# PhilipWilliamVentura/multimodal-financial-analysis-tool-using-paligemma

Measured on AMD Instinct MI355X. Metric: decode tokens/sec per GPU + prefill ms (224px img + 32-tok prompt), PaliGemma-3B, higher is better.
Workload: dtype bf16; 1 GPU; configs[1]: paligemma-3b-pt-224 greedy KV-cached decode, batch 1, after a 256-image-token + 32-text-token prefill; batch_per_gpu=1, global_batch=1, prompt_len=288, images_gathered=1, parallelism=replicas x1 (weights RCCL-broadcast), hipgraph=True, steps_per_graph_launch=1

## Files before the change

### include/pgmi.h

```cpp
#ifndef PGMI_H
#define PGMI_H

#include <stddef.h>
#include <stdint.h>

#ifdef __cplusplus
extern "C" {
#endif

#define PGMI_OK 0
#define PGMI_E_ARG -1
#define PGMI_E_STATE -2
#define PGMI_E_HIP -3
#define PGMI_E_NOMEM -4

#define PGMI_DTYPE_BF16 0
#define PGMI_DTYPE_F16 1
#define PGMI_DTYPE_F32 2

typedef struct pgmi_ctx pgmi_ctx;

typedef struct pgmi_config {
    int v_hidden, v_intermediate, v_layers, v_heads, v_channels, v_image, v_patch;
    float v_ln_eps;
// ... 54 lines not shown
                           const void* position, int position_dtype, const void* mask, int mask_dtype,
                           int64_t mask_b_stride, float* logits, int64_t* next_ids, int use_graph, void* stream);
int pgmi_set_prefill_graph(pgmi_ctx* ctx, int on);
#define PGMI_GRAPH_CACHE_MAX 64
int pgmi_graph_count(const pgmi_ctx* ctx, int which);
int pgmi_set_decode_staged_norm(pgmi_ctx* ctx, int on);
int pgmi_lm_head(pgmi_ctx* ctx, const void* normed, int rows, float* logits, void* stream);
int pgmi_lm_final_hidden(pgmi_ctx* ctx, void* out, int rows, void* stream);

#define PGMI_COMM_ID_BYTES 128
int pgmi_comm_unique_id(void* id_out);
int pgmi_comm_init(int device, int nranks, int rank, const void* id, void** comm_out);
int pgmi_comm_destroy(void* comm);
int pgmi_broadcast_weights(pgmi_ctx* ctx, void* comm, int root, void* stream);

int pgmi_argmax(pgmi_ctx* ctx, const float* logits, int rows, int V, int64_t* out, void* stream);

int pgmi_eos_update(pgmi_ctx* ctx, int64_t* next_ids, int32_t* finished, int B, int64_t eos_id, int64_t pad_id,
                    int32_t* n_alive, void* stream);

int pgmi_decode_kernel(pgmi_ctx* ctx, int which, int layer, int B, void* stream);

int pgmi_preprocess(pgmi_ctx* ctx, const void* src_hwc, int H, int W, int out_h, int out_w, float* out_chw,
                    void* stream);

int pgmi_prefill_kernel(pgmi_ctx* ctx, int which, int layer, int rows, void* stream);

int pgmi_prefill_probe(pgmi_ctx* ctx, int on);
int pgmi_prefill_probe_times(pgmi_ctx* ctx, float* us, int n);
int pgmi_tune_gemm(int cfg, int split);
int pgmi_tune_gemm_shape(int M, int N, int K, int dual, int cfg, int split);

int pgmi_debug_gemm_tiles(int n_mt, int n_nt, int S, int BM, int BN, int K, int* mt, int* nt, int* z);

int pgmi_tune_attention(int variant);

int pgmi_sample_top_p(pgmi_ctx* ctx, const float* x, int rows, int V, float temperature, float top_p,
                      const float* u, int64_t* out, float* kept_mass, void* stream);

int pgmi_op_gemm(pgmi_ctx* ctx, const void* A, const void* W, int M, int N, int K, int epi, const void* bias,
                 const void* res, void* out, void* stream);
int pgmi_op_gemm_strided(pgmi_ctx* ctx, const void* A, int lda, const void* W, int ldw, int M, int N, int K, int epi,
                         const void* bias, const void* res, void* out, void* stream);
int pgmi_op_rmsnorm(pgmi_ctx* ctx, const void* x, const void* w, int rows, int D, float eps, void* out,
                    void* stream);
int pgmi_op_layernorm(pgmi_ctx* ctx, const void* x, const void* w, const void* b, int rows, int D, float eps,
                      void* out, void* stream);
int pgmi_op_add(pgmi_ctx* ctx, const void* a, const void* b, int64_t n, void* out, void* stream);
int pgmi_op_patch_embed(pgmi_ctx* ctx, const void* pixels, int pixel_dtype, int B, int C, int H, int P,
                        const void* conv_w, const void* conv_b, const void* pos, int D, void* out, void* stream);
int pgmi_op_attention(pgmi_ctx* ctx, const void* q, const void* k, const void* v, void* o, int B, int Lq, int Lk,
                      int H, int Hkv, int head_dim, float scale, void* stream);
int pgmi_op_attention_ex(pgmi_ctx* ctx, const void* q, const void* k, const void* v, void* o, int B, int Lq, int Lk,
                         int H, int Hkv, int head_dim, int kv_layout, float scale, int scale_div, const void* mask,
                         int mask_dtype, int64_t m_b_stride, int64_t m_h_stride, int64_t m_q_stride, void* probs,
                         void* stream);
int pgmi_op_rope(pgmi_ctx* ctx, const void* x, const void* cos_rows, const void* sin_rows, int64_t rows, int heads,
                 int head_dim, void* out, void* stream);
int pgmi_op_scale(pgmi_ctx* ctx, const void* x, float a, int64_t n, void* out, void* stream);
int pgmi_op_gemv_res(pgmi_ctx* ctx, const void* x, const void* W, int B, int N, int K, void* h_inout,
                     void* stream);

#ifdef __cplusplus
}
#endif
#endif
// ... 1 lines not shown
```

### multimodal-financial-analysis-tool-using-paligemma_amd/csrc/engine.hip

```cpp
#include <algorithm>
#include <cmath>
#include <cstdio>
#include <cstdlib>
#include <cstring>
#include <map>
#include <string>
#include <unordered_map>
#include <vector>

#include <dlfcn.h>

#include <rccl/rccl.h>

#include "../../include/pgmi.h"
#include "common.h"
#include "launch.h"
#include "safetensors_hdr.h"

using namespace pgmi;

static thread_local std::string g_err;

static int fail(int code, const std::string& msg) {
    g_err = msg;
// ... 1355 lines not shown
    if ((rc = ensure_prepared(x))) return rc;
    const pgmi_config& c = x->c;
    if (rows < 1 || rows > c.max_batch * c.max_seq) return fail(PGMI_E_ARG, "rows exceed the prefill workspace");
    if (layer < 0 || layer >= c.t_layers) return fail(PGMI_E_ARG, "layer out of range");
    hipStream_t s = (hipStream_t)stream;
    const int H = c.t_hidden;
    const TextLayerW& w = x->w.t[layer];
    switch (which) {
        case 0: {
            EpiArgs g{};
            g.out = x->ACT; g.ldo = c.t_intermediate;
            gemm(s, x->Tn, H, w.gate_up, H, rows, c.t_intermediate, H, EPI_GEGLU, g, x->ws, x->ws_bytes,
                 c.t_intermediate);
            break;
        }
        case 1: {
            EpiArgs d{};
            d.res = x->Hs; d.ldr = H; d.out = x->Hs; d.ldo = H;
            gemm(s, x->ACT, c.t_intermediate, w.down, c.t_intermediate, rows, H, c.t_intermediate, EPI_RES, d, x->ws,
                 x->ws_bytes, 0, true);
            break;
        }
        default: return fail(PGMI_E_ARG, "unknown kernel id");
    }
    LAUNCHCHK();
    return 0;
}

int pgmi_debug_gemm_tiles(int n_mt, int n_nt, int S, int BM, int BN, int K, int* mt, int* nt, int* z) {
    if (n_mt < 1 || n_nt < 1 || S < 1 || !mt || !nt || !z) return fail(PGMI_E_ARG, "bad argument");
    return gemm_tile_order(n_mt, n_nt, S, BM, BN, K, mt, nt, z);
}

int pgmi_tune_gemm(int cfg, int split) {
    if (cfg >= kGemmCfgs || split < 0 || split > 32) return fail(PGMI_E_ARG, "bad GEMM plan");
    gemm_force_plan(cfg, split);
    return 0;
}

int pgmi_tune_gemm_shape(int M, int N, int K, int dual, int cfg, int split) {
    if (cfg >= kGemmCfgs || split < 0 || split > 16) return fail(PGMI_E_ARG, "bad GEMM plan");
    if (gemm_force_shape(M, N, K, dual, cfg, split)) return fail(PGMI_E_ARG, "too many per-shape GEMM plans");
    return 0;
}

int pgmi_tune_attention(int variant) {
    static const int ok[] = {-1, 0, 7, 8, 41, 42, 21, 22, 44, 24, 9, 91, 92, 94, 81, 82};
    for (int v : ok)
        if (v == variant) {
            attention_force_variant(variant);
            return 0;
        }
    return fail(PGMI_E_ARG, "unknown attention variant");
}

int pgmi_sample_top_p(pgmi_ctx* x, const float* logits, int rows, int V, float temperature, float top_p,
                      const float* u, int64_t* out, float* kept_mass, void* stream) {
    if (!x || !logits || !u || !out) return fail(PGMI_E_ARG, "null argument");
    if (rows <= 0 || V <= 0) return fail(PGMI_E_ARG, "sample_top_p: empty probabilities");
    if (!(top_p >= 0.f)) return fail(PGMI_E_ARG, "sample_top_p: top_p must be >= 0");
    if (!x->ws) return fail(PGMI_E_STATE, "workspace not allocated (pgmi_prepare)");
    const int per = (int)std::min<size_t>((size_t)rows, x->ws_bytes / sample_scratch_bytes(1, V));
    if (per < 1) return fail(PGMI_E_ARG, "sample_top_p: vocabulary exceeds the scratch");
    for (int r0 = 0; r0 < rows; r0 += per) {
        const int nr = std::min(per, rows - r0);
        sample_top_p((hipStream_t)stream, logits + (size_t)r0 * V, nr, V, temperature, top_p, u + r0, x->ws,
// ... 185 lines not shown
```

### multimodal-financial-analysis-tool-using-paligemma_amd/csrc/kernels_gemm.hip

```cpp
#include <map>
#include <mutex>
#include <tuple>
#include <vector>

#include <hip/hip_ext.h>

#include "common.h"
#include "launch.h"

#include <cstdlib>
#include <type_traits>

namespace pgmi {

constexpr int BK = 64;
constexpr int LDSK = 72;

#ifndef PGMI_GEMM_DIAG
#define PGMI_GEMM_DIAG 0
#endif
template <int TM, int TN, int NB>
__device__ __forceinline__ void diag_consume(const short8 (&fa)[TM], const short8 (&fb)[NB][TN]) {
#pragma unroll
    for (int i = 0; i < TM; ++i) asm volatile("" ::"v"(fa[i]));
#pragma unroll
    for (int b = 0; b < NB; ++b)
#pragma unroll
        for (int j = 0; j < TN; ++j) asm volatile("" ::"v"(fb[b][j]));
}

template <int EPI>
__device__ __forceinline__ void epi_store(const EpiArgs& ea, int m, int n, float acc, float acc2) {
// ... 1024 lines not shown
    P288w = 6,
    P256w = 7,
    P352w = 8,
    P288n = 9,
    P256n = 10,
    P128w = 11,
    P288t = 12,
    P256t = 13,
    P64x64 = 14,
    P128x64 = 15,
    P64x128 = 16,
    P128x128 = 17,
    P64x64d = 18,
    P128x64d = 19,
    Q288w = 20,
    Q352w = 21,
    Q256w = 22,
    Q288x256 = 23,
    P64x64s3 = 24,
    P64x64s4 = 25,
    P32x64s4 = 26,
    P64x32s4 = 27,
    P96x64s4 = 28,
    P96x64s3 = 29,
    W288w = 30,
    W288n = 31,
    W64x64 = 32,
    W352w = 33,
    W128x128 = 34,
    W128x64 = 35,
    E256 = 36,
    E192 = 37,
    R288w = 38,
    kNumCfg = 39,
};
static_assert(kNumCfg == kGemmCfgs, "launch.h kGemmCfgs");

struct Plan {
    Cfg cfg;
    int bm, bn, split;
};

static int g_force_cfg = -1, g_force_split = 0;

void gemm_force_plan(int cfg, int split) {
    g_force_cfg = cfg;
    g_force_split = split;
}

struct ShapePlan {
    int M, N, K;
    bool dual;
    int cfg, split;
};
static ShapePlan g_shape_plans[16];
static int g_n_shape_plans = 0;

int gemm_force_shape(int M, int N, int K, int dual, int cfg, int split) {
    for (int i = 0; i < g_n_shape_plans; ++i)
        if (g_shape_plans[i].M == M && g_shape_plans[i].N == N && g_shape_plans[i].K == K &&
            g_shape_plans[i].dual == (dual != 0)) {
            g_shape_plans[i] = g_shape_plans[--g_n_shape_plans];
            break;
        }
    if (cfg < 0) return 0;
    if (g_n_shape_plans >= 16) return -1;
    g_shape_plans[g_n_shape_plans++] = {M, N, K, dual != 0, cfg, split < 1 ? 1 : split};
    return 0;
}

static Plan choose(int M, int N, int K, bool dual) {
    if (g_force_cfg >= 0) {
        static const int bms[] = {288, 288, 256, 256, 128, 128, 288, 256, 352, 288, 256, 128, 288, 256, 64, 128, 64, 128, 64, 128, 288, 352, 256, 288, 64, 64, 32, 64, 96, 96, 288, 288, 64, 352, 128, 128, 256, 192, 288};
        static const int bns[] = {64, 32, 64, 32, 128, 64, 128, 128, 128, 64, 64, 128, 32, 32, 64, 64, 128, 128, 64, 64, 128, 128, 128, 256, 64, 64, 64, 32, 64, 64, 128, 64, 64, 128, 128, 64, 256, 256, 128};
        const int c = g_force_cfg;
        const int bn = (dual && c >= P288w) ? bns[c] / 2 : bns[c];
        return {(Cfg)c, bms[c], bn, dual && c < P288w ? 1 : (g_force_split > 0 ? g_force_split : 1)};
    }
    struct Entry { int M, N, K; bool dual; Cfg cfg; int split; };
    static const Entry table[] = {
        {288, 2560, 2048, false, W64x64, 1},
        {288, 2048, 2048, false, W128x128, 4},
        {288, 16384, 2048, true, R288w, 1},
        {288, 2048, 16384, false, W288n, 8},
        {256, 3456, 1152, false, P64x64s4, 1},
        {256, 1152, 1152, false, P64x64s4, 3},
        {256, 4304, 1152, false, P96x64s4, 1},
        {256, 1152, 4304, false, P96x64s4, 4},
        {256, 1152, 640, false, P64x32s4, 1},
        {256, 2048, 1152, false, P32x64s4, 1},
        {1056, 2560, 2048, false, W128x128, 1},
        {1056, 2048, 2048, false, W128x128, 1},
        {1056, 16384, 2048, true, E192, 1},
        {1056, 2048, 16384, false, E192, 5},
        {1024, 3456, 1152, false, W128x128, 1},
        {1024, 1152, 1152, false, P96x64s4, 1},
        {1024, 4304, 1152, false, W288w, 1},
        {1024, 1152, 4304, false, W128x128, 3},
        {2048, 3456, 1152, false, W288w, 1},
        {2048, 1152, 1152, false, W128x128, 1},
        {2048, 4304, 1152, false, W352w, 1},
        {2048, 1152, 4304, false, W288w, 2},
        {2048, 2048, 1152, false, W128x128, 1},
        {2304, 2560, 2048, false, Q256w, 1},
        {2304, 2048, 2048, false, W288n, 1},
        {2304, 16384, 2048, true, E256, 1},
        {2304, 2048, 16384, false, W288w, 2},
    };
    static const int bms[] = {288, 288, 256, 256, 128, 128, 288, 256, 352, 288, 256, 128, 288, 256, 64, 128, 64, 128, 64, 128, 288, 352, 256, 288, 64, 64, 32, 64, 96, 96, 288, 288, 64, 352, 128, 128, 256, 192, 288};
    static const int bns[] = {64, 32, 64, 32, 128, 64, 128, 128, 128, 64, 64, 128, 32, 32, 64, 64, 128, 128, 64, 64, 128, 128, 128, 256, 64, 64, 64, 32, 64, 64, 128, 64, 64, 128, 128, 64, 256, 256, 128};
    auto mk = [&](Cfg c, int split) -> Plan { return {c, bms[c], dual ? bns[c] / 2 : bns[c], dual ? 1 : split}; };
    for (int i = 0; i < g_n_shape_plans; ++i) {
        const ShapePlan& o = g_shape_plans[i];
        if (o.M == M && o.N == N && o.K == K && o.dual == dual) return mk((Cfg)o.cfg, o.split);
    }
    for (const Entry& e : table)
        if (e.M == M && e.N == N && e.K == K && e.dual == dual) return mk(e.cfg, e.split);
    if (M <= 16) {
        if (dual) return mk(P64x128, 1);
        if (K >= 8192) return mk(P64x64, 8);
    }
    if (dual) return mk(M <= 288 || M >= 2048 ? W288w : W352w, 1);
    if (K >= 8192) return mk(M <= 288 ? W288n : W288w, M <= 288 ? 8 : M <= 1056 ? 4 : 2);
    const long t64 = (long)((M + 63) / 64) * ((N + 63) / 64);
    if (t64 <= 256) return mk(P64x64, 1);
    const long t128 = (long)((M + 127) / 128) * ((N + 127) / 128);
    Plan p = mk(P128w, 1);
    const int nkt = (K + 63) / 64;
    while (t128 * p.split < 200 && p.split < 4 && nkt / (p.split * 2) >= 4) p.split *= 2;
    return p;
}

size_t gemm_ws_bytes(int M, int N, int K) {
    Plan p = choose(M, N, K, false);
    return p.split > 1 ? (size_t)p.split * M * N * sizeof(float) : 0;
}

static int xcd_block_pick(int n_mt, int n_nt, int S, int BM, int BN, int K);
static int xcd_block(int n_mt, int n_nt, int S, int BM, int BN, int K) {
    static std::mutex mu;
    static std::map<std::tuple<int, int, int, int, int, int>, int> memo;
    const auto key = std::make_tuple(n_mt, n_nt, S, BM, BN, K);
    std::lock_guard<std::mutex> lock(mu);
    auto it = memo.find(key);
    if (it != memo.end()) return it->second;
    const int code = xcd_block_pick(n_mt, n_nt, S, BM, BN, K);
    memo[key] = code;
    return code;
}

static int xcd_block_pick(int n_mt, int n_nt, int S, int BM, int BN, int K) {
    const long G = (long)n_mt * n_nt * S;
    if ((long)n_mt * BM < 2048) return 0;
    if (G % 8 != 0 || n_mt >= 64 * 8 || G > 65536) return 0;
    const double ks = (double)K / S * 2.0;
    const long q = G / 8;
    double run = 0.0;
    for (int x = 0; x < 8; ++x) {
        long na = 0, nb = 0;
        std::vector<char> sa((size_t)n_mt * S, 0), sb((size_t)n_nt * S, 0);
        for (long idx = x * q; idx < (x + 1) * q; ++idx) {
            const int mt = (int)(idx % n_mt), z = (int)((idx / n_mt) % S), nt = (int)(idx / ((long)n_mt * S));
            if (!sa[(size_t)mt * S + z]++) ++na;
            if (!sb[(size_t)nt * S + z]++) ++nb;
        }
        run += ks * ((double)na * BM + (double)nb * BN);
    }
    double best = 0.8 * run;
// ... 80 lines not shown
    const int n_mt = (M + BM - 1) / BM, n_nt = (N + BN - 1) / BN;
    dim3 grid(n_mt * n_nt, split);
    const int code = xcd_block(n_mt, n_nt, split, BM, NB * BN, K);
    static bool attr_set = false;
    if (!attr_set) {
        (void)hipFuncSetAttribute(reinterpret_cast<const void*>(&k_gemm_p<NW, WM, TM, TN, NB, STQ, EK, false>),
                                  hipFuncAttributeMaxDynamicSharedMemorySize, (int)lds);
        (void)hipFuncSetAttribute(reinterpret_cast<const void*>(&k_gemm_p<NW, WM, TM, TN, NB, STQ, EK, true>),
                                  hipFuncAttributeMaxDynamicSharedMemorySize, (int)lds);
        attr_set = true;
    }
    if (EPI < 0 || split > 1) {
        PGMI_GEMM_LAUNCH((k_gemm_p<NW, WM, TM, TN, NB, STQ, EK, true>), grid, dim3(64 * NW), lds, s, A, lda, W, ldw, M, N, K, per,
                           ea, ws, up_off, n_mt, code);
        if (EPI >= 0) {
            long total4 = ((long)M * N + 3) / 4;
            long blocks = (total4 + 255) / 256;
            if (blocks > 4096) blocks = 4096;
            hipLaunchKernelGGL((k_splitk_epi<EK>), dim3((unsigned)blocks), dim3(256), 0, s, ws, split, M, N, ea);
        }
    } else {
        PGMI_GEMM_LAUNCH((k_gemm_p<NW, WM, TM, TN, NB, STQ, EK, false>), grid, dim3(64 * NW), lds, s, A, lda, W, ldw, M, N, K,
                           per, ea, ws, up_off, n_mt, code);
    }
}

template <int NW, int WM, int TM, int TNW, int ST, int LW, int EPI, bool RL = false>
static void launch_w(hipStream_t s, const uint16_t* A, int lda, const uint16_t* W, int ldw, int M, int N, int K,
                     const EpiArgs& ea, float* ws, int split, long up_off) {
    constexpr bool DUAL = (EPI == EPI_GEGLU);
    constexpr int NB = DUAL ? 2 : 1;
    constexpr int TN = DUAL ? (TNW >= 2 ? TNW / 2 : 1) : TNW;
    constexpr int BM = WM * TM * 16, BN = (NW / WM) * TN * 16;
    constexpr size_t lds = (size_t)ST * (BM + NB * BN) * 128;
    static_assert(lds <= 163840, "LDS ring exceeds 160 KiB");
    constexpr int EK = EPI < 0 ? EPI_STORE : EPI;
    const int nkt = (K + 63) / 64;
    const int per = (nkt + split - 1) / split;
    const int n_mt = (M + BM - 1) / BM, n_nt = (N + BN - 1) / BN;
    dim3 grid(n_mt * n_nt, split);
    const int code = xcd_block(n_mt, n_nt, split, BM, NB * BN, K) | (n_mt == 1 ? 1 << 30 : 0);
    static bool attr_set = false;
    if (!attr_set) {
        (void)hipFuncSetAttribute(reinterpret_cast<const void*>(&k_gemm_w<NW, WM, TM, TN, NB, ST, LW, EK, false, RL>),
                                  hipFuncAttributeMaxDynamicSharedMemorySize, (int)lds);
        (void)hipFuncSetAttribute(reinterpret_cast<const void*>(&k_gemm_w<NW, WM, TM, TN, NB, ST, LW, EK, true, RL>),
                                  hipFuncAttributeMaxDynamicSharedMemorySize, (int)lds);
        attr_set = true;
    }
    const dim3 block(64 * (NW + LW));
    if (EPI < 0 || split > 1) {
        PGMI_GEMM_LAUNCH((k_gemm_w<NW, WM, TM, TN, NB, ST, LW, EK, true, RL>), grid, block, lds, s, A, lda, W, ldw, M, N, K,
                           per, ea, ws, up_off, n_mt, code);
        if (EPI >= 0) {
            long total4 = ((long)M * N + 3) / 4;
            long blocks = (total4 + 255) / 256;
            if (blocks > 4096) blocks = 4096;
            hipLaunchKernelGGL((k_splitk_epi<EK>), dim3((unsigned)blocks), dim3(256), 0, s, ws, split, M, N, ea);
        }
    } else {
        PGMI_GEMM_LAUNCH((k_gemm_w<NW, WM, TM, TN, NB, ST, LW, EK, false, RL>), grid, block, lds, s, A, lda, W, ldw, M, N, K,
                           per, ea, ws, up_off, n_mt, code);
    }
}

template <int TM, int EPI>
static void launch_8p(hipStream_t s, const uint16_t* A, int lda, const uint16_t* W, int ldw, int M, int N, int K,
                      const EpiArgs& ea, float* ws, int split, long up_off) {
    constexpr bool DUAL = (EPI == EPI_GEGLU);
    constexpr int BM = 32 * TM, BNO = DUAL ? 128 : 256;
    constexpr size_t lds = (size_t)2 * (2 * 16 * TM * 128 + 2 * 128 * 128);
    static_assert(lds <= 163840, "LDS exceeds 160 KiB");
    constexpr int EK = EPI < 0 ? EPI_STORE : EPI;
    const int nkt = K / 64;
    const int per = (nkt + split - 1) / split;
    const int n_mt = (M + BM - 1) / BM, n_nt = (N + BNO - 1) / BNO;
    dim3 grid(n_mt * n_nt, split);
    const int code = xcd_block(n_mt, n_nt, split, BM, DUAL ? 2 * BNO : BNO, K);
    static bool attr_set = false;
    if (!attr_set) {
        (void)hipFuncSetAttribute(reinterpret_cast<const void*>(&k_gemm_8p<TM, EK, false>),
                                  hipFuncAttributeMaxDynamicSharedMemorySize, (int)lds);
        (void)hipFuncSetAttribute(reinterpret_cast<const void*>(&k_gemm_8p<TM, EK, true>),
                                  hipFuncAttributeMaxDynamicSharedMemorySize, (int)lds);
        attr_set = true;
    }
    if (EPI < 0 || split > 1) {
        PGMI_GEMM_LAUNCH((k_gemm_8p<TM, EK, true>), grid, dim3(512), lds, s, A, lda, W, ldw, M, N, K, per, ea, ws,
                           up_off, n_mt, code);
        if (EPI >= 0) {
            long total4 = ((long)M * N + 3) / 4;
            long blocks = (total4 + 255) / 256;
            if (blocks > 4096) blocks = 4096;
            hipLaunchKernelGGL((k_splitk_epi<EK>), dim3((unsigned)blocks), dim3(256), 0, s, ws, split, M, N, ea);
// ... 13 lines not shown
        case P288w: P_(2, 9, 4, 3); break;
        case P256w: P_(2, 8, 4, 3); break;
        case P352w: P_(2, 11, 4, 2); break;
        case P288n: P_(2, 9, 2, 3); break;
        case P256n: P_(2, 8, 2, 4); break;
        case P128w: P_(2, 4, 4, 3); break;
        case P288t: P_(2, 9, 1, 4); break;
        case P256t: P_(4, 4, 2, 4); break;
        case P64x64: P_(2, 2, 2, 6); break;
        case P128x64: P_(2, 4, 2, 6); break;
        case P64x128: P_(2, 2, 4, 6); break;
        case P128x128: P_(2, 4, 4, 5); break;
        case P64x64d: P_(2, 2, 2, 10); break;
        case P128x64d: P_(4, 2, 4, 6); break;
        case Q288w: P8_(2, 9, 2, 3); break;
        case Q352w: P8_(2, 11, 2, 2); break;
        case Q256w: P8_(2, 8, 2, 3); break;
        case Q288x256: P8_(2, 9, 4, 2); break;
        case P64x64s3: P_(2, 2, 2, 3); break;
        case P64x64s4: P_(2, 2, 2, 4); break;
        case P32x64s4: P_(2, 1, 2, 4); break;
        case P64x32s4: P_(2, 2, 1, 4); break;
        case P96x64s4: P_(2, 3, 2, 4); break;
        case P96x64s3: P_(2, 3, 2, 3); break;
        case W288w: launch_w<8, 2, 9, 2, 3, 4, EPI>(s, A, lda, W, ldw, M, N, K, ea, ws, p.split, up_off); break;
        case W288n: launch_w<8, 2, 9, 1, 3, 4, EPI>(s, A, lda, W, ldw, M, N, K, ea, ws, p.split, up_off); break;
        case W64x64: launch_w<4, 2, 2, 2, 6, 4, EPI>(s, A, lda, W, ldw, M, N, K, ea, ws, p.split, up_off); break;
        case W352w: launch_w<8, 2, 11, 2, 2, 4, EPI>(s, A, lda, W, ldw, M, N, K, ea, ws, p.split, up_off); break;
        case W128x128: launch_w<8, 2, 4, 2, 4, 4, EPI>(s, A, lda, W, ldw, M, N, K, ea, ws, p.split, up_off); break;
        case W128x64: launch_w<4, 2, 4, 2, 5, 4, EPI>(s, A, lda, W, ldw, M, N, K, ea, ws, p.split, up_off); break;
        case E256: launch_8p<8, EPI>(s, A, lda, W, ldw, M, N, K, ea, ws, p.split, up_off); break;
        case E192: launch_8p<6, EPI>(s, A, lda, W, ldw, M, N, K, ea, ws, p.split, up_off); break;
        case R288w: launch_w<8, 2, 9, 2, 3, 4, EPI, true>(s, A, lda, W, ldw, M, N, K, ea, ws, p.split, up_off); break;
        default: break;
    }
#undef P_
#undef P8_
}

template <int EPI>
static void launch_e(hipStream_t s, const uint16_t* A, int lda, const uint16_t* W, int ldw, int M, int N, int K,
                     const EpiArgs& ea, float* ws, const Plan& p, long up_off) {
    switch (p.cfg) {
        case C288x64: launch_t<6, 1, 3, 4, EPI>(s, A, lda, W, ldw, M, N, K, ea, ws, p.split, up_off); break;
        case C288x32: launch_t<6, 1, 3, 2, EPI>(s, A, lda, W, ldw, M, N, K, ea, ws, p.split, up_off); break;
        case C256x64: launch_t<4, 1, 4, 4, EPI>(s, A, lda, W, ldw, M, N, K, ea, ws, p.split, up_off); break;
        case C256x32: launch_t<4, 1, 4, 2, EPI>(s, A, lda, W, ldw, M, N, K, ea, ws, p.split, up_off); break;
        case C128x128: launch_t<2, 2, 4, 4, EPI>(s, A, lda, W, ldw, M, N, K, ea, ws, p.split, up_off); break;
        case C128x64: launch_t<2, 2, 4, 2, EPI>(s, A, lda, W, ldw, M, N, K, ea, ws, p.split, up_off); break;
        default: launch_pcfg<EPI>(s, A, lda, W, ldw, M, N, K, ea, ws, p, up_off); break;
    }
}

int gemm(hipStream_t s, const uint16_t* A, int lda, const uint16_t* W, int ldw, int M, int N, int K, Epi epi,
         const EpiArgs& ea, float* ws, size_t ws_bytes, int up_offset_rows, bool defer) {
    Plan p = choose(M, N, K, epi == EPI_GEGLU);
    if ((p.cfg == E256 || p.cfg == E192) && K % 64 != 0) p.cfg = P128w;
    if (p.split > 1 && (size_t)p.split * M * N * sizeof(float) > ws_bytes) p.split = 1;
    if (p.split > 1 && N % 4 != 0) p.split = 1;
    const long up_off = (long)up_offset_rows * ldw;
    if (defer && p.split > 16) p.split = 16;
    if (p.split > 1) {
        const int nkt = (K + BK - 1) / BK;
        const int per = (nkt + p.split - 1) / p.split;
        p.split = (nkt + per - 1) / per;
    }
    if (defer && p.split > 1) {
        switch (p.cfg) {
            case C288x64: launch_t<6, 1, 3, 4, -1>(s, A, lda, W, ldw, M, N, K, ea, ws, p.split, up_off); break;
            case C288x32: launch_t<6, 1, 3, 2, -1>(s, A, lda, W, ldw, M, N, K, ea, ws, p.split, up_off); break;
            case C256x64: launch_t<4, 1, 4, 4, -1>(s, A, lda, W, ldw, M, N, K, ea, ws, p.split, up_off); break;
            case C256x32: launch_t<4, 1, 4, 2, -1>(s, A, lda, W, ldw, M, N, K, ea, ws, p.split, up_off); break;
            case C128x128: launch_t<2, 2, 4, 4, -1>(s, A, lda, W, ldw, M, N, K, ea, ws, p.split, up_off); break;
            case C128x64: launch_t<2, 2, 4, 2, -1>(s, A, lda, W, ldw, M, N, K, ea, ws, p.split, up_off); break;
            default: launch_pcfg<-1>(s, A, lda, W, ldw, M, N, K, ea, ws, p, up_off); break;
        }
        return p.split;
    }
    switch (epi) {
        case EPI_STORE: launch_e<EPI_STORE>(s, A, lda, W, ldw, M, N, K, ea, ws, p, up_off); break;
        case EPI_BIAS: launch_e<EPI_BIAS>(s, A, lda, W, ldw, M, N, K, ea, ws, p, up_off); break;
        case EPI_BIAS_GELU: launch_e<EPI_BIAS_GELU>(s, A, lda, W, ldw, M, N, K, ea, ws, p, up_off); break;
        case EPI_BIAS_RES: launch_e<EPI_BIAS_RES>(s, A, lda, W, ldw, M, N, K, ea, ws, p, up_off); break;
        case EPI_RES: launch_e<EPI_RES>(s, A, lda, W, ldw, M, N, K, ea, ws, p, up_off); break;
        case EPI_BIAS_POS: launch_e<EPI_BIAS_POS>(s, A, lda, W, ldw, M, N, K, ea, ws, p, up_off); break;
        case EPI_F32: launch_e<EPI_F32>(s, A, lda, W, ldw, M, N, K, ea, ws, p, up_off); break;
        case EPI_GEGLU: launch_e<EPI_GEGLU>(s, A, lda, W, ldw, M, N, K, ea, ws, p, up_off); break;
        case EPI_ROPE: return 0;
    }
    return 1;
}

bool gemm_qkv_rope(hipStream_t s, const uint16_t* A, int lda, const uint16_t* W, int ldw, int M, int N, int K,
                   const EpiArgs& ea) {
    if (N % 256 != 0 || N != (ea.nh + 2 * ea.nkv) * 256) return false;
    const Plan p = choose(M, N, K, false);
    if (p.split != 1) return false;
#define P_(wm, tm, st) launch_p<4, wm, tm, 2, st, EPI_ROPE>(s, A, lda, W, ldw, M, N, K, ea, nullptr, 1, 0)
#define W_(nw, tm, st) launch_w<nw, 2, tm, 2, st, 4, EPI_ROPE>(s, A, lda, W, ldw, M, N, K, ea, nullptr, 1, 0)
    switch (p.cfg) {
        case P288n: P_(2, 9, 3); break;
        case P64x64: P_(2, 2, 6); break;
        case P128x64: P_(2, 4, 6); break;
        case P64x64s3: P_(2, 2, 3); break;
        case P64x64s4: P_(2, 2, 4); break;
        case P32x64s4: P_(2, 1, 4); break;
        case P96x64s4: P_(2, 3, 4); break;
        case P96x64s3: P_(2, 3, 3); break;
        case W288w: W_(8, 9, 3); break;
        case W64x64: W_(4, 2, 6); break;
        case W352w: W_(8, 11, 2); break;
        case W128x128: W_(8, 4, 4); break;
        case W128x64: launch_w<4, 2, 4, 2, 5, 4, EPI_ROPE>(s, A, lda, W, ldw, M, N, K, ea, nullptr, 1, 0); break;
        default: return false;
    }
#undef P_
#undef W_
    return true;
}

int gemm_tile_order(int n_mt, int n_nt, int S, int BM, int BN, int K, int* mt, int* nt, int* z) {
    const int code = xcd_block(n_mt, n_nt, S, BM, BN, K);
    const int gx = n_mt * n_nt;
    for (int lin = 0; lin < gx * S; ++lin) xcd_tile_of(lin, gx, S, n_mt, code, mt[lin], nt[lin], z[lin]);
    return code;
}

#endif

// ... 2 lines not shown
```

### multimodal-financial-analysis-tool-using-paligemma_amd/csrc/launch.h

```cpp
#pragma once
#include <hip/hip_runtime.h>
#include <stdint.h>

namespace pgmi {

enum Epi : int {
    EPI_STORE = 0,
    EPI_BIAS = 1,
    EPI_BIAS_GELU = 2,
    EPI_BIAS_RES = 3,
    EPI_RES = 4,
    EPI_BIAS_POS = 5,
    EPI_F32 = 6,
    EPI_GEGLU = 7,
    EPI_ROPE = 8,
};

struct EpiArgs {
    const uint16_t* bias = nullptr;
    const uint16_t* res = nullptr;
    int ldr = 0;
    const uint16_t* pos = nullptr;
    int npos = 0;
    uint16_t* out = nullptr;
    int ldo = 0;
    float* out_f32 = nullptr;
    const int64_t* rpos = nullptr;
    const uint16_t* cosT = nullptr;
    const uint16_t* sinT = nullptr;
    int max_pos = 0;
    uint16_t* q_out = nullptr;
    uint16_t* kc = nullptr;
    uint16_t* vc = nullptr;
    long kv_b_stride = 0;
    int kv_start = 0;
    int L = 1;
    int nh = 0;
    int nkv = 0;
};

bool gemm_qkv_rope(hipStream_t s, const uint16_t* A, int lda, const uint16_t* W, int ldw, int M, int N, int K,
                   const EpiArgs& ea);
int gemm(hipStream_t s, const uint16_t* A, int lda, const uint16_t* W, int ldw, int M, int N, int K,
         Epi epi, const EpiArgs& ea, float* ws, size_t ws_bytes, int up_offset_rows = 0, bool defer = false);
size_t gemm_ws_bytes(int M, int N, int K);
void gemm_force_plan(int cfg, int split);
int gemm_force_shape(int M, int N, int K, int dual, int cfg, int split);
void gemm_probe_events(hipEvent_t start, hipEvent_t stop);
int gemm_tile_order(int n_mt, int n_nt, int S, int BM, int BN, int K, int* mt, int* nt, int* z);
constexpr int kGemmCfgs = 39;

struct StepState {
    int kv_len;
    int position;
};

struct EmbedFold {
    const int64_t* ids;
    const uint16_t* E;
    float normalizer;
    int64_t pad_id;
    uint16_t* h_out;
};
bool gemv_qkv_folds_embed(int B);
void gemv_qkv(hipStream_t s, int B, int nh, int nkv, const uint16_t* h, const uint16_t* norm_w, float eps,
              const uint16_t* Wqkv, const uint16_t* cosT, const uint16_t* sinT, int max_pos, const StepState* st,
              uint16_t* q_out, uint16_t* kc, uint16_t* vc, long kv_b_stride, float* ws = nullptr,
              const EmbedFold* emb = nullptr, const uint16_t* Wf = nullptr,
              int st_stride = 0);
void gemv_res(hipStream_t s, int B, int K, const uint16_t* x, const uint16_t* W, int N, uint16_t* h_inout,
              float* ws);
void gemv_res_norm(hipStream_t s, int B, int K, const uint16_t* x, const uint16_t* W, int N, uint16_t* h_inout,
                   float* ws, const uint16_t* norm_w, float eps, uint16_t* hn, const uint16_t* Wf = nullptr);
void mf_swizzle(hipStream_t s, const uint16_t* W, int rows, int K, uint16_t* out, bool qkv = false);
void rows_norm(hipStream_t s, const uint16_t* x, const uint16_t* w, float eps, int nb, int K, uint16_t* out);
void gemv_o_attn(hipStream_t s, int B, int G, const float* part, int max_chunks, const StepState* st,
                 const uint16_t* Wo, int N, uint16_t* h_inout, uint16_t* o_out, float* ssq = nullptr,
                 const uint16_t* Wf = nullptr, int st_stride = 0);
void gemv_geglu(hipStream_t s, int B, const uint16_t* h, const uint16_t* norm_w, float eps,
                const uint16_t* Wgu, int I, uint16_t* act, float* ssq = nullptr, const uint16_t* Wf = nullptr);
int gemv_logits_blocks();
int gemv_mf_min_batch();
bool gemv_logits(hipStream_t s, int B, const uint16_t* h, const uint16_t* norm_w, float eps,
// ... 94 lines not shown
```

### multimodal-financial-analysis-tool-using-paligemma_amd/pgmi/_native.py

```python
from __future__ import annotations

import ctypes
import os

import torch

_HERE = os.path.dirname(os.path.abspath(__file__))
LIB_PATH = os.environ.get("PGMI_LIB_PATH") or os.path.join(_HERE, "libpgmi.so")

PGMI_OK, PGMI_E_ARG, PGMI_E_STATE, PGMI_E_HIP, PGMI_E_NOMEM = 0, -1, -2, -3, -4
DTYPE_BF16, DTYPE_F16, DTYPE_F32 = 0, 1, 2

EPI = {"store": 0, "bias": 1, "bias_gelu": 2, "bias_res": 3, "res": 4, "bias_pos": 5, "f32": 6, "geglu": 7}


class PgmiConfig(ctypes.Structure):
    _fields_ = [
        ("v_hidden", ctypes.c_int), ("v_intermediate", ctypes.c_int), ("v_layers", ctypes.c_int),
        ("v_heads", ctypes.c_int), ("v_channels", ctypes.c_int), ("v_image", ctypes.c_int),
        ("v_patch", ctypes.c_int), ("v_ln_eps", ctypes.c_float),
        ("t_vocab", ctypes.c_int), ("t_hidden", ctypes.c_int), ("t_intermediate", ctypes.c_int),
        ("t_layers", ctypes.c_int), ("t_heads", ctypes.c_int), ("t_kv_heads", ctypes.c_int),
        ("t_head_dim", ctypes.c_int), ("t_max_pos", ctypes.c_int), ("t_rms_eps", ctypes.c_float),
        ("t_rope_theta", ctypes.c_float), ("projection_dim", ctypes.c_int),
# ... 11 lines not shown
    "pgmi_destroy": (i32, [vp]),
    "pgmi_weights_bytes": (i64, [vp]),
    "pgmi_weight_count": (i32, [vp]),
    "pgmi_weight_info": (i32, [vp, i32, ctypes.POINTER(ctypes.c_char_p), ctypes.POINTER(i64),
                               ctypes.POINTER(i64 * 4), ctypes.POINTER(i32)]),
    "pgmi_bind_weights": (i32, [vp, vp]),
    "pgmi_load_weight": (i32, [vp, ctypes.c_char_p, vp, i32, i32, vp]),
    "pgmi_fill_synthetic": (i32, [vp, ctypes.c_char_p, u64, f32, f32, vp]),
    "pgmi_load_safetensors": (i32, [vp, ctypes.c_char_p, ctypes.POINTER(i32), ctypes.POINTER(i32), vp]),
    "pgmi_safetensors_count": (i32, [ctypes.c_char_p, ctypes.POINTER(i32)]),
    "pgmi_safetensors_entry": (i32, [ctypes.c_char_p, i32, ctypes.c_char_p, i32, ctypes.POINTER(i32),
                                     ctypes.POINTER(i64 * 4), ctypes.POINTER(i32), ctypes.POINTER(i64),
                                     ctypes.POINTER(i64)]),
    "pgmi_synthetic_key": (u64, [ctypes.c_char_p, u64]),
    "pgmi_set_rope_inv_freq": (i32, [vp, ctypes.POINTER(f32)]),
    "pgmi_set_rope_table": (i32, [vp, vp, vp, i32]),
    "pgmi_prepare": (i32, [vp]),
    "pgmi_kv_bytes": (i64, [vp, i32, i32]),
    "pgmi_vision": (i32, [vp, vp, i32, i32, vp, vp]),
    "pgmi_project": (i32, [vp, vp, i32, vp, vp]),
    "pgmi_embed": (i32, [vp, vp, i32, vp, vp]),
    "pgmi_lm_forward": (i32, [vp, vp, vp, i32, vp, i32, i32, vp, vp, i32, i32, i32, vp, i32, vp]),
    "pgmi_decode": (i32, [vp, vp, i32, vp, i32, i32, i32, i32, vp, vp, i32, vp]),
    "pgmi_decode_steps": (i32, [vp, vp, i32, vp, i32, i32, i32, i32, i32, vp, vp, i32, vp]),
    "pgmi_lm_forward_ragged": (i32, [vp, vp, vp, i32, vp, i32, i32, vp, vp, vp, i32, i32, i32, vp, i32, vp]),
    "pgmi_decode_ragged": (i32, [vp, vp, i32, vp, i32, i32, vp, vp, i32, vp, vp, vp, i32, vp]),
    "pgmi_decode_embeds": (i32, [vp, vp, i32, vp, i32, i32, i32, i32, vp, vp, i32, vp]),
    "pgmi_decode_embeds_dev": (i32, [vp, vp, i32, vp, i32, i32, i32, vp, i32, vp, i32, i64, vp, vp, i32, vp]),
    "pgmi_set_prefill_graph": (i32, [vp, i32]),
    "pgmi_graph_count": (i32, [vp, i32]),
    "pgmi_set_decode_staged_norm": (i32, [vp, i32]),
    "pgmi_prefill_kernel": (i32, [vp, i32, i32, i32, vp]),
    "pgmi_debug_gemm_tiles": (i32, [i32, i32, i32, i32, i32, i32, vp, vp, vp]),
    "pgmi_prefill_probe": (i32, [vp, i32]),
    "pgmi_prefill_probe_times": (i32, [vp, ctypes.POINTER(f32), i32]),
    "pgmi_preprocess": (i32, [vp, vp, i32, i32, i32, i32, vp, vp]),
    "pgmi_argmax": (i32, [vp, vp, i32, i32, vp, vp]),
    "pgmi_lm_head": (i32, [vp, vp, i32, vp, vp]),
    "pgmi_lm_final_hidden": (i32, [vp, vp, i32, vp]),
    "pgmi_comm_unique_id": (i32, [vp]),
    "pgmi_comm_init": (i32, [i32, i32, i32, vp, ctypes.POINTER(vp)]),
    "pgmi_comm_destroy": (i32, [vp]),
    "pgmi_broadcast_weights": (i32, [vp, vp, i32, vp]),
    "pgmi_eos_update": (i32, [vp, vp, vp, i32, i64, i64, vp, vp]),
    "pgmi_decode_kernel": (i32, [vp, i32, i32, i32, vp]),
    "pgmi_tune_gemm": (i32, [i32, i32]),
    "pgmi_tune_gemm_shape": (i32, [i32, i32, i32, i32, i32, i32]),
    "pgmi_tune_attention": (i32, [i32]),
    "pgmi_sample_top_p": (i32, [vp, vp, i32, i32, f32, f32, vp, vp, vp, vp]),
    "pgmi_op_gemm": (i32, [vp, vp, vp, i32, i32, i32, i32, vp, vp, vp, vp]),
    "pgmi_op_gemm_strided": (i32, [vp, vp, i32, vp, i32, i32, i32, i32, i32, vp, vp, vp, vp]),
    "pgmi_op_rmsnorm": (i32, [vp, vp, vp, i32, i32, f32, vp, vp]),
    "pgmi_op_layernorm": (i32, [vp, vp, vp, vp, i32, i32, f32, vp, vp]),
    "pgmi_op_attention": (i32, [vp, vp, vp, vp, vp, i32, i32, i32, i32, i32, i32, f32, vp]),
    "pgmi_op_add": (i32, [vp, vp, vp, i64, vp, vp]),
    "pgmi_op_patch_embed": (i32, [vp, vp, i32, i32, i32, i32, i32, vp, vp, vp, i32, vp, vp]),
    "pgmi_op_gemv_res": (i32, [vp, vp, vp, i32, i32, i32, vp, vp]),
    "pgmi_op_attention_ex": (i32, [vp, vp, vp, vp, vp, i32, i32, i32, i32, i32, i32, i32, f32, i32, vp, i32, i64, i64,
                                   i64, vp, vp]),
    "pgmi_op_rope": (i32, [vp, vp, vp, vp, i64, i32, i32, vp, vp]),
    "pgmi_op_scale": (i32, [vp, vp, f32, i64, vp, vp]),
}

_lib = None


# ... 56 lines not shown
```

Before: 806.5 tokens/s.

## Choose GEMM tile and split-K via analytic cost model for untabled shapes

Replaces the heuristic GEMM plan fallback for M>16 with two steps: first reuse the plan of the nearest tabled shape that has the same tile count, otherwise score candidate tile configs and split-K factors with a simple model of staging bytes, CU rounds and split-K slab traffic. Adds a new 352x64 tile config, clamps the LDS pipeline stage count so larger tiles fit in 160 KiB, and exposes a debug entry point to query the chosen plan. Decode (M<=16) keeps its existing rules, so the change mainly targets prefill GEMM shapes. The risk is that the model picks worse plans than the old heuristics for some shapes.

```diff
diff --git a/include/pgmi.h b/include/pgmi.h
--- a/include/pgmi.h
+++ b/include/pgmi.h
@@ -110,6 +110,7 @@
 int pgmi_tune_gemm_shape(int M, int N, int K, int dual, int cfg, int split);
 
 int pgmi_debug_gemm_tiles(int n_mt, int n_nt, int S, int BM, int BN, int K, int* mt, int* nt, int* z);
+int pgmi_debug_gemm_plan(int M, int N, int K, int dual, int* cfg, int* split, int* bm, int* bn);
 
 int pgmi_tune_attention(int variant);
 
diff --git a/multimodal-financial-analysis-tool-using-paligemma_amd/csrc/engine.hip b/multimodal-financial-analysis-tool-using-paligemma_amd/csrc/engine.hip
--- a/multimodal-financial-analysis-tool-using-paligemma_amd/csrc/engine.hip
+++ b/multimodal-financial-analysis-tool-using-paligemma_amd/csrc/engine.hip
@@ -1411,6 +1411,13 @@
     return gemm_tile_order(n_mt, n_nt, S, BM, BN, K, mt, nt, z);
 }
 
+int pgmi_debug_gemm_plan(int M, int N, int K, int dual, int* cfg, int* split, int* bm, int* bn) {
+    if (M < 1 || N < 1 || K < 1 || dual < 0 || dual > 3 || !cfg || !split || !bm || !bn)
+        return fail(PGMI_E_ARG, "bad argument");
+    gemm_plan(M, N, K, dual, cfg, split, bm, bn);
+    return 0;
+}
+
 int pgmi_tune_gemm(int cfg, int split) {
     if (cfg >= kGemmCfgs || split < 0 || split > 32) return fail(PGMI_E_ARG, "bad GEMM plan");
     gemm_force_plan(cfg, split);
diff --git a/multimodal-financial-analysis-tool-using-paligemma_amd/csrc/kernels_gemm.hip b/multimodal-financial-analysis-tool-using-paligemma_amd/csrc/kernels_gemm.hip
--- a/multimodal-financial-analysis-tool-using-paligemma_amd/csrc/kernels_gemm.hip
+++ b/multimodal-financial-analysis-tool-using-paligemma_amd/csrc/kernels_gemm.hip
@@ -1,3 +1,5 @@
+#include <cmath>
+#include <iterator>
 #include <map>
 #include <mutex>
 #include <tuple>
@@ -1088,9 +1090,24 @@
     E256 = 36,
     E192 = 37,
     R288w = 38,
-    kNumCfg = 39,
+    W352n = 39,
+    kNumCfg = 40,
 };
 static_assert(kNumCfg == kGemmCfgs, "launch.h kGemmCfgs");
+
+struct Tile {
+    int bm, bn;
+};
+static const Tile kTiles[kNumCfg] = {
+    {288, 64},  {288, 32},  {256, 64},  {256, 32},  {128, 128}, {128, 64},
+    {288, 128}, {256, 128}, {352, 128}, {288, 64},  {256, 64},  {128, 128}, {288, 32},  {256, 32},
+    {64, 64},   {128, 64},  {64, 128},  {128, 128}, {64, 64},   {128, 64},
+    {288, 128}, {352, 128}, {256, 128}, {288, 256},
+    {64, 64},   {64, 64},   {32, 64},   {64, 32},   {96, 64},   {96, 64},
+    {288, 128}, {288, 64},  {64, 64},   {352, 128}, {128, 128}, {128, 64},
+    {256, 256}, {192, 256},
+    {288, 128}, {352, 64},
+};
 
 struct Plan {
     Cfg cfg;
@@ -1125,13 +1142,57 @@
     return 0;
 }
 
-static Plan choose(int M, int N, int K, bool dual) {
+constexpr double kModelCUs = 256.0;
+constexpr double kIntakeBytesPerUs = 43e3;
+constexpr double kStreamBytesPerUs = 7.2e6;
+constexpr size_t kModelWsBytes = (size_t)64 << 20;
+constexpr double kCombineLaunchUs = 4.0;
+constexpr int kModelMinKTiles = 8;
+
+static double model_us(int M, int N, int K, bool dual, bool deferred, Cfg c, int split) {
+    const Tile t = kTiles[c];
+    const int nkt = (K + 63) / 64, per = (nkt + split - 1) / split;
+    const long n_mt = (M + t.bm - 1) / t.bm, n_nt = (N + (dual ? t.bn / 2 : t.bn) - 1) / (dual ? t.bn / 2 : t.bn);
+    const double rounds = std::ceil((double)(n_mt * n_nt * split) / kModelCUs);
+    const double staged = 128.0 * per * (t.bm + t.bn);
+    const double slabs = split > 1 ? 2.0 * split * M * N * sizeof(float) : 0.0;
+    return rounds * staged / kIntakeBytesPerUs + slabs / kStreamBytesPerUs + (split > 1 && !deferred ? kCombineLaunchUs : 0.0);
+}
+
+static void model_plan(int M, int N, int K, bool dual, bool unsplit, bool deferred, Cfg& best_c, int& best_s) {
+    static const Cfg kDual[] = {R288w, W288w, W352w, E192, E256};
+    static const Cfg kPlain[] = {W64x64, W128x64, W128x128, W288n, W352n, W288w, W352w, E192, E256};
+    static const Cfg kRope[] = {W64x64, W128x64, W128x128, W288w, W352w};
+    static const int kSplits[] = {1, 2, 3, 4, 5, 6, 8};
+    const Cfg* list = dual ? kDual : unsplit ? kRope : kPlain;
+    const int n = (int)(dual ? std::size(kDual) : unsplit ? std::size(kRope) : std::size(kPlain));
+    const int nkt = (K + 63) / 64;
+    double best = 0.0;
+    bool have = false;
+    for (int i = 0; i < n; ++i) {
+        const Cfg c = list[i];
+        if ((c == E192 || c == E256) && K % 64 != 0) continue;
+        for (int split : kSplits) {
+            if (split > 1) {
+                if (dual || unsplit || N % 4 != 0) break;
+                const int per = (nkt + split - 1) / split;
+                if (per < kModelMinKTiles || (nkt + per - 1) / per != split) continue;
+                if ((size_t)split * M * N * sizeof(float) > kModelWsBytes) break;
+            }
+            const double us = model_us(M, N, K, dual, deferred, c, split);
+            if (!have || us < best) { best = us; best_c = c; best_s = split; have = true; }
+        }
+    }
+}
+
+static Plan choose(int M, int N, int K, bool dual, bool unsplit = false, bool deferred = false) {
+    auto mk = [&](Cfg c, int split) -> Plan {
+        return {c, kTiles[c].bm, dual ? kTiles[c].bn / 2 : kTiles[c].bn, dual ? 1 : split};
+    };
     if (g_force_cfg >= 0) {
-        static const int bms[] = {288, 288, 256, 256, 128, 128, 288, 256, 352, 288, 256, 128, 288, 256, 64, 128, 64, 128, 64, 128, 288, 352, 256, 288, 64, 64, 32, 64, 96, 96, 288, 288, 64, 352, 128, 128, 256, 192, 288};
-        static const int bns[] = {64, 32, 64, 32, 128, 64, 128, 128, 128, 64, 64, 128, 32, 32, 64, 64, 128, 128, 64, 64, 128, 128, 128, 256, 64, 64, 64, 32, 64, 64, 128, 64, 64, 128, 128, 64, 256, 256, 128};
         const int c = g_force_cfg;
-        const int bn = (dual && c >= P288w) ? bns[c] / 2 : bns[c];
-        return {(Cfg)c, bms[c], bn, dual && c < P288w ? 1 : (g_force_split > 0 ? g_force_split : 1)};
+        const int bn = (dual && c >= P288w) ? kTiles[c].bn / 2 : kTiles[c].bn;
+        return {(Cfg)c, kTiles[c].bm, bn, dual && c < P288w ? 1 : (g_force_split > 0 ? g_force_split : 1)};
     }
     struct Entry { int M, N, K; bool dual; Cfg cfg; int split; };
     static const Entry table[] = {
@@ -1163,9 +1224,6 @@
         {2304, 16384, 2048, true, E256, 1},
         {2304, 2048, 16384, false, W288w, 2},
     };
-    static const int bms[] = {288, 288, 256, 256, 128, 128, 288, 256, 352, 288, 256, 128, 288, 256, 64, 128, 64, 128, 64, 128, 288, 352, 256, 288, 64, 64, 32, 64, 96, 96, 288, 288, 64, 352, 128, 128, 256, 192, 288};
-    static const int bns[] = {64, 32, 64, 32, 128, 64, 128, 128, 128, 64, 64, 128, 32, 32, 64, 64, 128, 128, 64, 64, 128, 128, 128, 256, 64, 64, 64, 32, 64, 64, 128, 64, 64, 128, 128, 64, 256, 256, 128};
-    auto mk = [&](Cfg c, int split) -> Plan { return {c, bms[c], dual ? bns[c] / 2 : bns[c], dual ? 1 : split}; };
     for (int i = 0; i < g_n_shape_plans; ++i) {
         const ShapePlan& o = g_shape_plans[i];
         if (o.M == M && o.N == N && o.K == K && o.dual == dual) return mk((Cfg)o.cfg, o.split);
@@ -1175,21 +1233,39 @@
     if (M <= 16) {
         if (dual) return mk(P64x128, 1);
         if (K >= 8192) return mk(P64x64, 8);
-    }
-    if (dual) return mk(M <= 288 || M >= 2048 ? W288w : W352w, 1);
-    if (K >= 8192) return mk(M <= 288 ? W288n : W288w, M <= 288 ? 8 : M <= 1056 ? 4 : 2);
-    const long t64 = (long)((M + 63) / 64) * ((N + 63) / 64);
-    if (t64 <= 256) return mk(P64x64, 1);
-    const long t128 = (long)((M + 127) / 128) * ((N + 127) / 128);
-    Plan p = mk(P128w, 1);
-    const int nkt = (K + 63) / 64;
-    while (t128 * p.split < 200 && p.split < 4 && nkt / (p.split * 2) >= 4) p.split *= 2;
-    return p;
+        const long t64 = (long)((M + 63) / 64) * ((N + 63) / 64);
+        if (t64 <= 256) return mk(P64x64, 1);
+        const long t128 = (long)((M + 127) / 128) * ((N + 127) / 128);
+        Plan p = mk(P128w, 1);
+        const int nkt = (K + 63) / 64;
+        while (t128 * p.split < 200 && p.split < 4 && nkt / (p.split * 2) >= 4) p.split *= 2;
+        return p;
+    }
+    const Entry* near = nullptr;
+    for (const Entry& e : table) {
+        const int bm = kTiles[e.cfg].bm;
+        if (e.N == N && e.K == K && e.dual == dual && M < e.M && (M + bm - 1) / bm == (e.M + bm - 1) / bm &&
+            (!near || e.M < near->M))
+            near = &e;
+    }
+    if (near) return mk(near->cfg, near->split);
+    Cfg c = W64x64;
+    int split = 1;
+    model_plan(M, N, K, dual, unsplit, deferred, c, split);
+    return mk(c, split);
 }
 
 size_t gemm_ws_bytes(int M, int N, int K) {
     Plan p = choose(M, N, K, false);
     return p.split > 1 ? (size_t)p.split * M * N * sizeof(float) : 0;
+}
+
+void gemm_plan(int M, int N, int K, int kind, int* cfg, int* split, int* bm, int* bn) {
+    const Plan p = choose(M, N, K, kind == 1, kind == 2, kind == 3);
+    *cfg = p.cfg;
+    *split = p.split;
+    *bm = p.bm;
+    *bn = p.bn;
 }
 
 static int xcd_block_pick(int n_mt, int n_nt, int S, int BM, int BN, int K);
@@ -1336,7 +1412,8 @@
     constexpr int NB = DUAL ? 2 : 1;
     constexpr int TN = DUAL ? (TNW >= 2 ? TNW / 2 : 1) : TNW;
     constexpr int BM = WM * TM * 16, BN = (NW / WM) * TN * 16;
-    constexpr size_t lds = (size_t)ST * (BM + NB * BN) * 128;
+    constexpr int STQ = (size_t)ST * (BM + NB * BN) * 128 <= 163840 ? ST : ST - 1;
+    constexpr size_t lds = (size_t)STQ * (BM + NB * BN) * 128;
     static_assert(lds <= 163840, "LDS ring exceeds 160 KiB");
     constexpr int EK = EPI < 0 ? EPI_STORE : EPI;
     const int nkt = (K + 63) / 64;
@@ -1346,15 +1423,15 @@
     const int code = xcd_block(n_mt, n_nt, split, BM, NB * BN, K) | (n_mt == 1 ? 1 << 30 : 0);
     static bool attr_set = false;
     if (!attr_set) {
-        (void)hipFuncSetAttribute(reinterpret_cast<const void*>(&k_gemm_w<NW, WM, TM, TN, NB, ST, LW, EK, false, RL>),
+        (void)hipFuncSetAttribute(reinterpret_cast<const void*>(&k_gemm_w<NW, WM, TM, TN, NB, STQ, LW, EK, false, RL>),
                                   hipFuncAttributeMaxDynamicSharedMemorySize, (int)lds);
-        (void)hipFuncSetAttribute(reinterpret_cast<const void*>(&k_gemm_w<NW, WM, TM, TN, NB, ST, LW, EK, true, RL>),
+        (void)hipFuncSetAttribute(reinterpret_cast<const void*>(&k_gemm_w<NW, WM, TM, TN, NB, STQ, LW, EK, true, RL>),
                                   hipFuncAttributeMaxDynamicSharedMemorySize, (int)lds);
         attr_set = true;
     }
     const dim3 block(64 * (NW + LW));
     if (EPI < 0 || split > 1) {
-        PGMI_GEMM_LAUNCH((k_gemm_w<NW, WM, TM, TN, NB, ST, LW, EK, true, RL>), grid, block, lds, s, A, lda, W, ldw, M, N, K,
+        PGMI_GEMM_LAUNCH((k_gemm_w<NW, WM, TM, TN, NB, STQ, LW, EK, true, RL>), grid, block, lds, s, A, lda, W, ldw, M, N, K,
                            per, ea, ws, up_off, n_mt, code);
         if (EPI >= 0) {
             long total4 = ((long)M * N + 3) / 4;
@@ -1363,7 +1440,7 @@
             hipLaunchKernelGGL((k_splitk_epi<EK>), dim3((unsigned)blocks), dim3(256), 0, s, ws, split, M, N, ea);
         }
     } else {
-        PGMI_GEMM_LAUNCH((k_gemm_w<NW, WM, TM, TN, NB, ST, LW, EK, false, RL>), grid, block, lds, s, A, lda, W, ldw, M, N, K,
+        PGMI_GEMM_LAUNCH((k_gemm_w<NW, WM, TM, TN, NB, STQ, LW, EK, false, RL>), grid, block, lds, s, A, lda, W, ldw, M, N, K,
                            per, ea, ws, up_off, n_mt, code);
     }
 }
@@ -1443,6 +1520,7 @@
         case E256: launch_8p<8, EPI>(s, A, lda, W, ldw, M, N, K, ea, ws, p.split, up_off); break;
         case E192: launch_8p<6, EPI>(s, A, lda, W, ldw, M, N, K, ea, ws, p.split, up_off); break;
         case R288w: launch_w<8, 2, 9, 2, 3, 4, EPI, true>(s, A, lda, W, ldw, M, N, K, ea, ws, p.split, up_off); break;
+        case W352n: launch_w<8, 2, 11, 1, 3, 4, EPI>(s, A, lda, W, ldw, M, N, K, ea, ws, p.split, up_off); break;
         default: break;
     }
 #undef P_
@@ -1465,7 +1543,7 @@
 
 int gemm(hipStream_t s, const uint16_t* A, int lda, const uint16_t* W, int ldw, int M, int N, int K, Epi epi,
          const EpiArgs& ea, float* ws, size_t ws_bytes, int up_offset_rows, bool defer) {
-    Plan p = choose(M, N, K, epi == EPI_GEGLU);
+    Plan p = choose(M, N, K, epi == EPI_GEGLU, false, defer);
     if ((p.cfg == E256 || p.cfg == E192) && K % 64 != 0) p.cfg = P128w;
     if (p.split > 1 && (size_t)p.split * M * N * sizeof(float) > ws_bytes) p.split = 1;
     if (p.split > 1 && N % 4 != 0) p.split = 1;
@@ -1505,7 +1583,7 @@
 bool gemm_qkv_rope(hipStream_t s, const uint16_t* A, int lda, const uint16_t* W, int ldw, int M, int N, int K,
                    const EpiArgs& ea) {
     if (N % 256 != 0 || N != (ea.nh + 2 * ea.nkv) * 256) return false;
-    const Plan p = choose(M, N, K, false);
+    const Plan p = choose(M, N, K, false, true);
     if (p.split != 1) return false;
 #define P_(wm, tm, st) launch_p<4, wm, tm, 2, st, EPI_ROPE>(s, A, lda, W, ldw, M, N, K, ea, nullptr, 1, 0)
 #define W_(nw, tm, st) launch_w<nw, 2, tm, 2, st, 4, EPI_ROPE>(s, A, lda, W, ldw, M, N, K, ea, nullptr, 1, 0)
diff --git a/multimodal-financial-analysis-tool-using-paligemma_amd/csrc/launch.h b/multimodal-financial-analysis-tool-using-paligemma_amd/csrc/launch.h
--- a/multimodal-financial-analysis-tool-using-paligemma_amd/csrc/launch.h
+++ b/multimodal-financial-analysis-tool-using-paligemma_amd/csrc/launch.h
@@ -44,11 +44,12 @@
 int gemm(hipStream_t s, const uint16_t* A, int lda, const uint16_t* W, int ldw, int M, int N, int K,
          Epi epi, const EpiArgs& ea, float* ws, size_t ws_bytes, int up_offset_rows = 0, bool defer = false);
 size_t gemm_ws_bytes(int M, int N, int K);
+void gemm_plan(int M, int N, int K, int kind, int* cfg, int* split, int* bm, int* bn);
 void gemm_force_plan(int cfg, int split);
 int gemm_force_shape(int M, int N, int K, int dual, int cfg, int split);
 void gemm_probe_events(hipEvent_t start, hipEvent_t stop);
 int gemm_tile_order(int n_mt, int n_nt, int S, int BM, int BN, int K, int* mt, int* nt, int* z);
-constexpr int kGemmCfgs = 39;
+constexpr int kGemmCfgs = 40;
 
 struct StepState {
     int kv_len;
diff --git a/multimodal-financial-analysis-tool-using-paligemma_amd/pgmi/_native.py b/multimodal-financial-analysis-tool-using-paligemma_amd/pgmi/_native.py
--- a/multimodal-financial-analysis-tool-using-paligemma_amd/pgmi/_native.py
+++ b/multimodal-financial-analysis-tool-using-paligemma_amd/pgmi/_native.py
@@ -67,6 +67,7 @@
     "pgmi_set_decode_staged_norm": (i32, [vp, i32]),
     "pgmi_prefill_kernel": (i32, [vp, i32, i32, i32, vp]),
     "pgmi_debug_gemm_tiles": (i32, [i32, i32, i32, i32, i32, i32, vp, vp, vp]),
+    "pgmi_debug_gemm_plan": (i32, [i32, i32, i32, i32, vp, vp, vp, vp]),
     "pgmi_prefill_probe": (i32, [vp, i32]),
     "pgmi_prefill_probe_times": (i32, [vp, ctypes.POINTER(f32), i32]),
     "pgmi_preprocess": (i32, [vp, vp, i32, i32, i32, i32, vp, vp]),
```

Result: no change. 805.2 tokens/s (-0.2%).
